# raymondclowe/EasyWakeWord

Hardware: AMD Instinct MI355X
Metric: real-time 16 kHz streams sustained + MFCC frames/sec at 1/2/4/8 GPUs (higher is better)
Workload: dtype fp32

## Files before the change

### easywakeword_amd/csrc/ewk_mfcc.hip

```cpp
#include <hip/hip_runtime.h>
#include <math.h>

#include "ewk_internal.h"
#include "ewk_score.h"
#include "ewk_db64.h"
#include "ewk_topdb_shift.h"
#include "ewk_rs_list.h"

#define EWK_SETPRIO(v) __builtin_amdgcn_s_setprio(v)

#ifdef EWK_TIMING
#define EWK_DBG_PARAM , uint64_t(&dbg)[kDbgN]
#define EWK_DBG_ARG , dbg
#define EWK_TS(v) const uint64_t v = __builtin_amdgcn_s_memtime()
#define EWK_TADD(k, a, b) dbg[k] += (b) - (a)
#define EWK_PASS_PARAM , uint64_t* pdbg
#define EWK_PASS_ARG(x) , x
#else
#define EWK_DBG_PARAM
#define EWK_DBG_ARG
#define EWK_TS(v)
#define EWK_TADD(k, a, b)
#define EWK_PASS_PARAM
#define EWK_PASS_ARG(x)
#endif
#ifdef EWK_TIMING
constexpr int kDbgN = 24;
#endif

namespace ewk {

#ifdef EWK_TIMING
__device__ unsigned long long g_ewk_dbg[kDbgN];
#endif
#ifdef EWK_LIST_STATS
__device__ unsigned long long g_ewk_list[10];
#endif
#ifdef EWK_COOP_DEBUG
constexpr int kCoopKeys = 32 * 256;
__device__ int4 g_coop_ev[kCoopKeys][WAVES];
__device__ float4 g_coop_th[kCoopKeys][WAVES];
__device__ double g_coop_pd[kCoopKeys][WAVES][60];
__device__ float g_coop_ms[kCoopKeys][40];
__device__ uint4 g_coop_tile[4 * 256][WAVES][512];
#define EWK_COOP_KEY_PARAM , int dkey
#define EWK_COOP_KEY_ARG(k) , (k)
#else
#define EWK_COOP_KEY_PARAM
#define EWK_COOP_KEY_ARG(k)
#endif

typedef float floatx4 __attribute__((ext_vector_type(4)));

constexpr int kFPP = 4 * kNF;
constexpr int kStageLoads = ((kFPP - 1) * HOP + NFFT + 63) / 64;
constexpr int kScrFrames = kFPP * SCR_FRAME + 8 * (kNF - 1);
__host__ __device__ constexpr int stg_off(int c) { return 256 * c + 128 * (c / 5); }
__host__ __device__ constexpr int win_off(int g, int n1) {
    return 4 * (160 * g + 32 * n1 + 32 * ((160 * g + 32 * n1) / 320));
}
constexpr int kStageFloats = stg_off(kStageLoads) / 4;
constexpr int kScrFloats = (kScrFrames > kStageFloats) ? kScrFrames : kStageFloats;
constexpr int SCR_BYTES = (kScrFloats * 4 + 15) & ~15;
constexpr int L_SCR = 0;
constexpr int L_TAB = L_SCR + WAVES * SCR_BYTES;
static_assert(L_SCR + (WAVES - 1) * SCR_BYTES < 65536, "ds_write_addtid_b32 bases must fit M0[15:0]");

constexpr int TP = 18;
constexpr int WP = 52;
constexpr int L_WIN2 = L_TAB;
constexpr int L_TW1 = L_WIN2 + 16 * TP * 8;
constexpr int L_TW2 = L_TW1 + 16 * TP * 8;
constexpr int L_WPAD = L_TW2 + 16 * TP * 8;
constexpr int L_BLO = L_WPAD + 16 * WP * 4;
constexpr int L_DCT = L_BLO + NMEL * 4;
constexpr float kDctScale = 1024.0f;
constexpr float kTopDbUnits = 80.0f;
constexpr int DCT_RT1 = 4 * 2 * 64 * 16;
constexpr int DCT_RT1_STRIDE = 17 * 16;
constexpr int kSlots = 5;
constexpr int DCT_BYTES = DCT_RT1 + 8 * DCT_RT1_STRIDE;
constexpr int L_SHARED_END = ((L_DCT + DCT_BYTES) + 15) & ~15;
constexpr int W_TILE = 0;
constexpr int kSpecTiles = 48;
constexpr int W_SPEC = W_TILE + 16 * NMEL * 4;
constexpr int kSpecRun = (16 / kFPP) * kSpecTiles;
constexpr int kSpecOrder = kSpecRun + kSpecTiles;
constexpr int W_BYTES = W_SPEC + (kSpecOrder + kSpecTiles) * 4;
static_assert(W_BYTES % 16 == 0 && kSpecTiles <= 64, "per-wave LDS carve; one bit per recorded tile");
constexpr int L_WG = L_SHARED_END + WAVES * W_BYTES;
constexpr int LDS_BYTES = L_WG + 16 + 8 * WAVES;
#ifndef EWK_TINY_MEAN
#define EWK_TINY_MEAN 32.0
#endif
constexpr double kTinyMean = EWK_TINY_MEAN;
#ifndef EWK_NAN_MARGIN_A
#define EWK_NAN_MARGIN_A 0.5
#endif
constexpr double kNanMarginA = EWK_NAN_MARGIN_A;
constexpr double kNanMarginB = 0.05;
static_assert(LDS_BYTES <= 160 * 1024, "the workgroup must fit a CU's LDS");
static_assert(16 % kFPP == 0, "passes must tile the 16-frame log-mel tile");


__device__ __forceinline__ void lds_order() { asm volatile("" ::: "memory"); }

#define EWK_LD128(r, a, c) asm volatile("ds_read_b128 %0, %1 offset:%2" : "=v"(r[c]) : "v"(a), "i"(16 * (c)) : "memory")
#define EWK_LD128_8(r, addr)                                                                        \
    do {                                                                                           \
        const uint32_t _a = (addr);                                                                \
        EWK_LD128(r, _a, 0); EWK_LD128(r, _a, 1); EWK_LD128(r, _a, 2); EWK_LD128(r, _a, 3);         \
        EWK_LD128(r, _a, 4); EWK_LD128(r, _a, 5); EWK_LD128(r, _a, 6); EWK_LD128(r, _a, 7);         \
    } while (0)
#define EWK_WAIT_8(r)                                                                              \
    asm volatile("s_waitcnt lgkmcnt(0)" : "+v"(r[0]), "+v"(r[1]), "+v"(r[2]), "+v"(r[3]), "+v"(r[4]), \
                 "+v"(r[5]), "+v"(r[6]), "+v"(r[7]) : : "memory")

__device__ __forceinline__ float2 cmul(float2 a, float2 w) {
    return make_float2(a.x * w.x - a.y * w.y, a.x * w.y + a.y * w.x);
}

__device__ __forceinline__ void dft4(float2& a0, float2& a1, float2& a2, float2& a3) {
    const float2 t0 = make_float2(a0.x + a2.x, a0.y + a2.y);
    const float2 t1 = make_float2(a0.x - a2.x, a0.y - a2.y);
    const float2 t2 = make_float2(a1.x + a3.x, a1.y + a3.y);
    const float2 t3 = make_float2(a1.x - a3.x, a1.y - a3.y);
    a0 = make_float2(t0.x + t2.x, t0.y + t2.y);
    a2 = make_float2(t0.x - t2.x, t0.y - t2.y);
    a1 = make_float2(t1.x + t3.y, t1.y - t3.x);
    a3 = make_float2(t1.x - t3.y, t1.y + t3.x);
}

__device__ __forceinline__ void dft16_stage2(float2 (&x)[16]) {
    constexpr float C1 = 0.92387953251128674f, R2 = 0.70710678118654752f, T = 0.41421356237309505f;
    dft4(x[0], x[1], x[2], x[3]);
    {
        const float2 a0 = x[4], y1 = x[5], y2 = x[6], y3 = x[7];
        const float2 u2 = make_float2(y2.x + y2.y, y2.y - y2.x);
        const float2 t0 = make_float2(fmaf(R2, u2.x, a0.x), fmaf(R2, u2.y, a0.y));
        const float2 t1 = make_float2(fmaf(-R2, u2.x, a0.x), fmaf(-R2, u2.y, a0.y));
        const float2 u1 = make_float2(fmaf(T, y1.y, y1.x), fmaf(-T, y1.x, y1.y));
        const float2 u3 = make_float2(fmaf(T, y3.x, y3.y), fmaf(T, y3.y, -y3.x));
        const float2 v2 = make_float2(u1.x + u3.x, u1.y + u3.y), v3 = make_float2(u1.x - u3.x, u1.y - u3.y);
        x[4] = make_float2(fmaf(C1, v2.x, t0.x), fmaf(C1, v2.y, t0.y));
        x[6] = make_float2(fmaf(-C1, v2.x, t0.x), fmaf(-C1, v2.y, t0.y));
        x[5] = make_float2(fmaf(C1, v3.y, t1.x), fmaf(-C1, v3.x, t1.y));
        x[7] = make_float2(fmaf(-C1, v3.y, t1.x), fmaf(C1, v3.x, t1.y));
    }
    {
        const float2 a0 = x[8], y1 = x[9], y2 = x[10], y3 = x[11];
        const float2 t0 = make_float2(a0.x + y2.y, a0.y - y2.x);
        const float2 t1 = make_float2(a0.x - y2.y, a0.y + y2.x);
        const float2 u1 = make_float2(y1.x + y1.y, y1.y - y1.x);
        const float d3 = y3.y - y3.x, n3 = y3.x + y3.y;
        const float2 v2 = make_float2(u1.x + d3, u1.y - n3), v3 = make_float2(u1.x - d3, u1.y + n3);
        x[8] = make_float2(fmaf(R2, v2.x, t0.x), fmaf(R2, v2.y, t0.y));
        x[10] = make_float2(fmaf(-R2, v2.x, t0.x), fmaf(-R2, v2.y, t0.y));
        x[9] = make_float2(fmaf(R2, v3.y, t1.x), fmaf(-R2, v3.x, t1.y));
        x[11] = make_float2(fmaf(-R2, v3.y, t1.x), fmaf(R2, v3.x, t1.y));
    }
    {
        const float2 a0 = x[12], y1 = x[13], y2 = x[14], y3 = x[15];
        const float d2 = y2.y - y2.x, n2 = y2.x + y2.y;
        const float2 t0 = make_float2(fmaf(R2, d2, a0.x), fmaf(-R2, n2, a0.y));
        const float2 t1 = make_float2(fmaf(-R2, d2, a0.x), fmaf(R2, n2, a0.y));
        const float2 u1 = make_float2(fmaf(T, y1.x, y1.y), fmaf(T, y1.y, -y1.x));
        const float m3 = fmaf(T, y3.y, y3.x), u3y = fmaf(T, y3.x, -y3.y);
        const float2 v2 = make_float2(u1.x - m3, u1.y + u3y), v3 = make_float2(u1.x + m3, u1.y - u3y);
        x[12] = make_float2(fmaf(C1, v2.x, t0.x), fmaf(C1, v2.y, t0.y));
        x[14] = make_float2(fmaf(-C1, v2.x, t0.x), fmaf(-C1, v2.y, t0.y));
        x[13] = make_float2(fmaf(C1, v3.y, t1.x), fmaf(-C1, v3.x, t1.y));
        x[15] = make_float2(fmaf(-C1, v3.y, t1.x), fmaf(C1, v3.x, t1.y));
    }
}

__device__ __forceinline__ void dft16_perm(float2 (&x)[16]) {
#pragma unroll
    for (int n2 = 0; n2 < 4; ++n2) dft4(x[n2], x[4 + n2], x[8 + n2], x[12 + n2]);
    dft16_stage2(x);
}
// ... 295 lines not shown
                    }
                }
            }
            lds_order();
        }
    }
    EWK_TS(fp3);
    EWK_SETPRIO(0);
#pragma unroll
    for (int g = 0; g < kNF; ++g) dft16_perm(b[g]);
    EWK_TS(fp4);
    {
        const bool z0 = jp == 0;
        float2 tw[18];
        {
            const float4* t4 = reinterpret_cast<const float4*>(smem + L_TW2) + jp * (TP / 2);
#pragma unroll
            for (int c = 0; c < 9; ++c) {
                const float4 q = t4[c];
                tw[2 * c] = make_float2(q.x, q.y);
                tw[2 * c + 1] = make_float2(q.z, q.w);
            }
        }
        float* pA0 = scf + rowA;
        float* pA1 = z0 ? scf - 136 : pA0;
        float* pA2 = z0 ? scf - 136 : pA0 - 16;
        float* pB0 = scf - rowA;
        float* pB1 = z0 ? scf + 136 : pB0;
        float* pB2 = z0 ? scf + 136 : pB0 + 16;
#pragma unroll
        for (int it0 = 0; it0 < 17; it0 += 2) {
            float py[2], px[2];
#pragma unroll
            for (int u = 0; u < 2; ++u) {
                const int it = it0 + u;
                if (it >= 17) break;
                const float2 w = tw[it];
                const float2 ug = b[0][dperm(it < 16 ? it : 15)];
                const float2 vg = b[1][dperm(it < 16 ? 15 - it : 0)];
                float2 uu, vv;
                if (it <= 8) {
                    uu = ug;
                    const float2 vz = b[0][dperm((16 - it) & 15)];
                    vv = z0 ? vz : vg;
                } else {
                    const float2 uz = b[1][dperm(it - 9)], vz = b[1][dperm(24 - it)];
                    uu = z0 ? uz : ug;
                    vv = z0 ? vz : vg;
                }
                const float ar = uu.x + vv.x, ai = uu.y - vv.y;
                const float br = uu.x - vv.x, bi = uu.y + vv.y;
                const float er = fmaf(w.y, br, -bi), ei = fmaf(w.y, bi, br);
                const float yr = fmaf(-w.x, er, ar), yi = fmaf(-w.x, ei, ai);
                const float xr = fmaf(w.x, er, ar), xi = fmaf(w.x, ei, ai);
                py[u] = yr * yr + yi * yi;
                px[u] = xr * xr + xi * xi;
            }
#pragma unroll
            for (int u = 0; u < 2; ++u) {
                const int it = it0 + u;
                if (it >= 17) break;
                float* pa = it <= 8 ? pA0 : (it < 16 ? pA1 : pA2);
                pa[16 * it] = py[u];
            }
#pragma unroll
            for (int u = 0; u < 2; ++u) {
                const int it = it0 + u;
                if (it >= 17) break;
                float* pb = it <= 8 ? pB0 : (it < 16 ? pB1 : pB2);
                pb[256 - 16 * it] = px[u];
            }
        }
        scf[257 + jp] = 0.0f;
        if (jp < 7) scf[265 + jp] = 0.0f;
    }
    lds_order();
    EWK_TS(fp5);
    EWK_SETPRIO(1);
    if (next_t0 >= 0) stage_load(v, next_t0 * HOP - NFFT / 2, lane, pf);
    float db[kNF][8];
    {
        const float* wrow = reinterpret_cast<const float*>(smem + L_WPAD) + j * WP;
#pragma unroll
        for (int hh = 0; hh < 2; ++hh) {
            const int i0 = hh ? 6 : 0, i1 = hh ? 8 : 6;
            float wv[MEL_ITERS], pv[kNF][MEL_ITERS];
#pragma unroll
            for (int i = i0; i < i1; ++i) {
                if (kMelW[i] <= 2) {
                    const float2 w = *reinterpret_cast<const float2*>(wrow + kMelOff[i]);
                    wv[kMelIt0[i]] = w.x; wv[kMelIt0[i] + 1] = w.y;
                } else {
#pragma unroll
                    for (int c = 0; c < (kMelW[i] + 3) / 4; ++c) {
                        const float4 w = *reinterpret_cast<const float4*>(wrow + kMelOff[i] + 4 * c);
                        const float ww[4] = {w.x, w.y, w.z, w.w};
#pragma unroll
                        for (int e = 0; e < 4; ++e)
                            if (4 * c + e < kMelW[i]) wv[kMelIt0[i] + 4 * c + e] = ww[e];
                    }
                }
#pragma unroll
                for (int g = 0; g < kNF; ++g) {
                    const float* sp = sc[g] + lo[i];
#pragma unroll
                    for (int q = 0; q < kMelW[i]; ++q) pv[g][kMelIt0[i] + q] = sp[q];
                }
            }
#pragma unroll
            for (int i = i0; i < i1; ++i)
#pragma unroll
                for (int g = 0; g < kNF; ++g) {
                    float acc = 0.0f;
#pragma unroll
                    for (int q = 0; q < kMelW[i]; ++q) acc = fmaf(wv[kMelIt0[i] + q], pv[g][kMelIt0[i] + q], acc);
                    db[g][i] = 3.0102999566398120f * __log2f(fmaxf(1e-10f, acc));
                    if (i == 0) nanp = fmaf(acc, 0.0f, nanp);
                }
        }
    }
    EWK_SETPRIO(0);
    lds_order();
    EWK_TS(fp6);
#pragma unroll
    for (int g = 0; g < kNF; ++g) {
        const int r = row0 + 2 * f + g;
        float fmx = db[g][0], fmn = db[g][0], x[8];
#pragma unroll
        for (int i = 0; i < 8; ++i) {
            fmx = fmaxf(fmx, db[g][i]);
            fmn = fminf(fmn, db[g][i]);
            x[i] = fmaxf(db[g][i], clampv);
        }
        vmax = fmaxf(vmax, valid[g] ? fmx : -INFINITY);
        vmin = fminf(vmin, valid[g] ? fmn : INFINITY);
        uint4 hi, lo;
        split8(x, hi, lo);
        unsigned char* tb = reinterpret_cast<unsigned char*>(tile) + tile_chunk(r, j);
        *reinterpret_cast<uint4*>(tb) = hi;
        *reinterpret_cast<uint4*>(tb + 256) = lo;
    }
    lds_order();
    if (next_t0 >= 0) stage_store(scr, lane, pf);
    lds_order();
#ifdef EWK_TIMING
    EWK_TS(fp7);
    if (pdbg) {
        pdbg[12] += fp1 - fp0; pdbg[13] += fp2 - fp1; pdbg[14] += fp3 - fp2; pdbg[15] += fp4 - fp3;
        pdbg[16] += fp5 - fp4; pdbg[17] += fp6 - fp5; pdbg[18] += fp7 - fp6; pdbg[19] += 1;
    }
#endif
}

#define EWK_DCT_RD(dst, addr, off) asm volatile("ds_read_b128 %0, %1 offset:%2" : "=v"(dst) : "v"(addr), "i"(off) : "memory")
#define EWK_DCT_LOAD(p, q)                                                   \
    do {                                                                     \
        EWK_DCT_RD(Bh[p], bq[q], 0);                                         \
        EWK_DCT_RD(Bl[p], bq[q], 256);                                       \
        EWK_DCT_RD(A0h[p], a0, 2048 * (q));                                  \
        EWK_DCT_RD(A0l[p], a0, 2048 * (q) + 1024);                           \
        EWK_DCT_RD(A1h[p], a1, DCT_RT1_STRIDE * (2 * (q)));                  \
        EWK_DCT_RD(A1l[p], a1, DCT_RT1_STRIDE * (2 * (q) + 1));              \
    } while (0)
#define EWK_DCT_WAIT(p, n)                                                                               \
    asm volatile("s_waitcnt lgkmcnt(" #n ")"                                                             \
                 : "+v"(Bh[p]), "+v"(Bl[p]), "+v"(A0h[p]), "+v"(A0l[p]), "+v"(A1h[p]), "+v"(A1l[p]) \
                 :                                                                                       \
                 : "memory")
#define EWK_MF(a, b, acc) \
    acc = __builtin_amdgcn_mfma_f32_16x16x32_f16(__builtin_bit_cast(halfx8, a), __builtin_bit_cast(halfx8, b), acc, 0, 0, 0)
#define EWK_DCT_MFMA(p)                                                                        \
    do {                                                                                       \
        EWK_MF(A0h[p], Bh[p], acc0); EWK_MF(A1h[p], Bh[p], acc1);                              \
        EWK_MF(A0h[p], Bl[p], acc0); EWK_MF(A1h[p], Bl[p], acc1);                              \
        EWK_MF(A0l[p], Bh[p], acc0); EWK_MF(A1l[p], Bh[p], acc1);                              \
        if (MASK) {                                                                            \
            const floatx4 mk = clamp_mask(Bh[p], Bl[p], cp, mnab);                             \
            EWK_MF(A0h[p], mk, am0); EWK_MF(A1h[p], mk, am1);                                  \
            EWK_MF(A0l[p], mk, am0); EWK_MF(A1l[p], mk, am1);                                  \
        }                                                                                      \
    } while (0)

__device__ __forceinline__ float pair_sum_lo(uint32_t h, uint32_t l) {
    float r;
    asm("v_fma_mix_f32 %0, %1, 1.0, %2 op_sel_hi:[1,0,1]" : "=v"(r) : "v"(h), "v"(l));
    return r;
}
__device__ __forceinline__ float pair_sum_hi(uint32_t h, uint32_t l) {
    float r;
    asm("v_fma_mix_f32 %0, %1, 1.0, %2 op_sel:[1,0,1] op_sel_hi:[1,0,1]" : "=v"(r) : "v"(h), "v"(l));
    return r;
}
struct ClampPair {
    uint32_t h2, l2;
    float eff;
};
__device__ __forceinline__ ClampPair clamp_pair(float clampv) {
    ClampPair cp;
    split2(clampv, clampv, cp.h2, cp.l2);
    cp.eff = pair_sum_lo(cp.h2, cp.l2);
    return cp;
}
__device__ __forceinline__ floatx4 clamp_mask(floatx4 bh, floatx4 bl, const ClampPair& cp, float& mn) {
    const uint4 h = __builtin_bit_cast(uint4, bh), l = __builtin_bit_cast(uint4, bl);
    const uint32_t hw[4] = {h.x, h.y, h.z, h.w}, lw[4] = {l.x, l.y, l.z, l.w};
    const uint32_t ones = 0x00010001u;
    uint32_t mw[4];
#pragma unroll
    for (int k = 0; k < 4; ++k) {
        const uint32_t t = (hw[k] ^ cp.h2) | (lw[k] ^ cp.l2);
        uint32_t u, zm;
        asm("v_pk_min_u16 %0, %1, %2" : "=v"(u) : "v"(t), "s"(ones));
        asm("v_pk_sub_u16 %0, %1, %2" : "=v"(zm) : "v"(u), "s"(ones));
        mw[k] = zm & 0x3C003C00u;
        const uint32_t hm = (zm & 0x7C007C00u) | (hw[k] & ~zm);
        asm("v_min3_f32 %0, %0, %1, %2" : "+v"(mn) : "v"(pair_sum_lo(hm, lw[k])), "v"(pair_sum_hi(hm, lw[k])));
    }
    return __builtin_bit_cast(floatx4, make_uint4(mw[0], mw[1], mw[2], mw[3]));
}

template <bool MASK>
__device__ __forceinline__ void tile_dct_m(const float* tile, const float* s_dct, int lane, float (&c)[kSlots],
                                           float (&m)[kSlots], float& mnab, const ClampPair& cp) {
    const int col = lane & 15, g4 = lane >> 4;
    floatx4 acc0 = {0.f, 0.f, 0.f, 0.f}, acc1 = {0.f, 0.f, 0.f, 0.f};
    floatx4 am0 = {0.f, 0.f, 0.f, 0.f}, am1 = {0.f, 0.f, 0.f, 0.f};
    const uint32_t tb = (uint32_t)(uintptr_t)tile + 512 * col + 16 * (g4 ^ (col & 3));
    uint32_t bq[4];
#pragma unroll
    for (int q = 0; q < 4; ++q) bq[q] = tb + 64 * (q ^ (col >> 2));
    const uint32_t db = (uint32_t)(uintptr_t)s_dct;
    const uint32_t a0 = db + 16 * lane;
    const uint32_t a1 = db + DCT_RT1 + 16 * ((col & 3) == 0 ? 4 * g4 + (col >> 2) : 16);
    floatx4 Bh[2], Bl[2], A0h[2], A0l[2], A1h[2], A1l[2];
    EWK_DCT_LOAD(0, 0);
    EWK_DCT_LOAD(1, 1);
    EWK_DCT_WAIT(0, 6);
    EWK_DCT_MFMA(0);
    EWK_DCT_LOAD(0, 2);
    EWK_DCT_WAIT(1, 6);
    EWK_DCT_MFMA(1);
    EWK_DCT_LOAD(1, 3);
    EWK_DCT_WAIT(0, 6);
    EWK_DCT_MFMA(0);
    EWK_DCT_WAIT(1, 0);
    EWK_DCT_MFMA(1);
    lds_order();
#pragma unroll
    for (int i = 0; i < 4; ++i) c[i] = acc0[i] * (1.0f / kDctScale);
    c[4] = acc1[0] * (1.0f / kDctScale);
    if (MASK) {
#pragma unroll
        for (int i = 0; i < 4; ++i) m[i] = am0[i] * (1.0f / kDctScale);
        m[4] = am1[0] * (1.0f / kDctScale);
    }
}
__device__ __forceinline__ void tile_dct(const float* tile, const float* s_dct, int lane, float (&c)[kSlots]) {
    float m[kSlots], mnab = 0.0f;
    tile_dct_m<false>(tile, s_dct, lane, c, m, mnab, ClampPair{0u, 0u, 0.0f});
}
#undef EWK_DCT_RD
#undef EWK_DCT_LOAD
#undef EWK_DCT_WAIT
#undef EWK_DCT_MFMA
#undef EWK_MF

__device__ __forceinline__ void stats_add(const float (&c)[kSlots], const float (&cref)[kSlots], bool ok, double (&s1)[kSlots],
                                          double (&s2)[kSlots]) {
    if (ok) {
#pragma unroll
        for (int i = 0; i < kSlots; ++i) {
            const double d = (double)c[i] - (double)cref[i];
            s1[i] += d;
            s2[i] = fma(d, d, s2[i]);
        }
    }
}

__device__ __forceinline__ void stats_replace(const float (&cn)[kSlots], const float (&co)[kSlots], const float (&cref)[kSlots],
                                              bool ok, double (&s1)[kSlots], double (&s2)[kSlots]) {
    if (ok) {
#pragma unroll
        for (int i = 0; i < kSlots; ++i) {
            const double dn = (double)cn[i] - (double)cref[i], dd = (double)co[i] - (double)cref[i];
            s1[i] += dn - dd;
            s2[i] += fma(dn, dn, -dd * dd);
        }
    }
}

__device__ __forceinline__ void shift_tile_add(const float (&c)[kSlots], const float (&cref)[kSlots],
                                               const float (&m)[kSlots], bool ok, float (&sA)[kSlots],
                                               float (&sB)[kSlots], float (&sC)[kSlots]) {
    if (ok) {
#pragma unroll
        for (int i = 0; i < kSlots; ++i) shift_add<float, float>(c[i] - cref[i], m[i], sA[i], sB[i], sC[i]);
    }
}
__device__ __forceinline__ void shift_apply(double delta, const float (&sA)[kSlots], float (&sB)[kSlots],
                                            const float (&sC)[kSlots], double (&s1)[kSlots], double (&s2)[kSlots]) {
#pragma unroll
    for (int i = 0; i < kSlots; ++i) shift_rise<float, float>(delta, sA[i], sB[i], sC[i], s1[i], s2[i]);
}
__device__ __forceinline__ void stats_replace_shift(const float (&cn)[kSlots], const float (&co)[kSlots], const float (&m)[kSlots],
                                                    double delta, const float (&cref)[kSlots], bool ok, double (&s1)[kSlots],
                                                    double (&s2)[kSlots]) {
    if (ok) {
#pragma unroll
        for (int i = 0; i < kSlots; ++i)
            shift_replace((double)cn[i], (double)co[i], (double)m[i], delta, (double)cref[i], s1[i], s2[i]);
    }
}

__device__ __forceinline__ void pass_mins(float x, float (&pm)[2]) {
    x = fminf(x, __int_as_float(__builtin_amdgcn_update_dpp(__float_as_int(x), __float_as_int(x), 0x111, 0xf, 0xf, false)));
    x = fminf(x, __int_as_float(__builtin_amdgcn_update_dpp(__float_as_int(x), __float_as_int(x), 0x112, 0xf, 0xf, false)));
    x = fminf(x, __int_as_float(__builtin_amdgcn_update_dpp(__float_as_int(x), __float_as_int(x), 0x114, 0xf, 0xf, false)));
#pragma unroll
    for (int p = 0; p < 2; ++p) {
        const float r0 = __int_as_float(__builtin_amdgcn_readlane(__float_as_int(x), 7 + 8 * p));
        const float r1 = __int_as_float(__builtin_amdgcn_readlane(__float_as_int(x), 23 + 8 * p));
        const float r2 = __int_as_float(__builtin_amdgcn_readlane(__float_as_int(x), 39 + 8 * p));
        const float r3 = __int_as_float(__builtin_amdgcn_readlane(__float_as_int(x), 55 + 8 * p));
        pm[p] = fminf(fminf(r0, r1), fminf(r2, r3));
    }
}

__device__ __forceinline__ float wave_min(float x) {
    x = fminf(x, __int_as_float(__builtin_amdgcn_update_dpp(__float_as_int(x), __float_as_int(x), 0x111, 0xf, 0xf, false)));
    x = fminf(x, __int_as_float(__builtin_amdgcn_update_dpp(__float_as_int(x), __float_as_int(x), 0x112, 0xf, 0xf, false)));
    x = fminf(x, __int_as_float(__builtin_amdgcn_update_dpp(__float_as_int(x), __float_as_int(x), 0x114, 0xf, 0xf, false)));
    x = fminf(x, __int_as_float(__builtin_amdgcn_update_dpp(__float_as_int(x), __float_as_int(x), 0x118, 0xf, 0xf, false)));
    const float r0 = __int_as_float(__builtin_amdgcn_readlane(__float_as_int(x), 15));
    const float r1 = __int_as_float(__builtin_amdgcn_readlane(__float_as_int(x), 31));
    const float r2 = __int_as_float(__builtin_amdgcn_readlane(__float_as_int(x), 47));
    const float r3 = __int_as_float(__builtin_amdgcn_readlane(__float_as_int(x), 63));
    return fminf(fminf(r0, r1), fminf(r2, r3));
}

template <int CTRL>
__device__ __forceinline__ double dpp_d(double x) {
    const int lo = __builtin_amdgcn_update_dpp(0, __double2loint(x), CTRL, 0xf, 0xf, false);
    const int hi = __builtin_amdgcn_update_dpp(0, __double2hiint(x), CTRL, 0xf, 0xf, false);
    return __hiloint2double(hi, lo);
}

__device__ __forceinline__ double row_sum_d(double x) {
    x += dpp_d<0x111>(x);
    x += dpp_d<0x112>(x);
    x += dpp_d<0x114>(x);
    x += dpp_d<0x118>(x);
    return x;
}

__device__ __forceinline__ double wave_sum_d(double x) {
    x = row_sum_d(x);
    double t = 0.0;
#pragma unroll
    for (int r = 0; r < 4; ++r)
        t += __hiloint2double(__builtin_amdgcn_readlane(__double2hiint(x), 16 * r + 15),
                              __builtin_amdgcn_readlane(__double2loint(x), 16 * r + 15));
    return t;
}

__device__ __forceinline__ float wave_sum_f(float x) {
    x += __int_as_float(__builtin_amdgcn_update_dpp(0, __float_as_int(x), 0x111, 0xf, 0xf, false));
    x += __int_as_float(__builtin_amdgcn_update_dpp(0, __float_as_int(x), 0x112, 0xf, 0xf, false));
    x += __int_as_float(__builtin_amdgcn_update_dpp(0, __float_as_int(x), 0x114, 0xf, 0xf, false));
    x += __int_as_float(__builtin_amdgcn_update_dpp(0, __float_as_int(x), 0x118, 0xf, 0xf, false));
    return (__int_as_float(__builtin_amdgcn_readlane(__float_as_int(x), 15)) +
            __int_as_float(__builtin_amdgcn_readlane(__float_as_int(x), 31))) +
           (__int_as_float(__builtin_amdgcn_readlane(__float_as_int(x), 47)) +
            __int_as_float(__builtin_amdgcn_readlane(__float_as_int(x), 63)));
}

__device__ __forceinline__ float wave_max(float x) { return -wave_min(-x); }

__device__ __forceinline__ void finish_stats(int T, const float (&cref)[kSlots], double (&s1)[kSlots], double (&s2)[kSlots],
                                             int lane, double* pd) {
#pragma unroll
    for (int i = 0; i < kSlots; ++i) {
        s1[i] = row_sum_d(s1[i]);
        s2[i] = row_sum_d(s2[i]);
    }
    if ((lane & 15) == 15) {
        const int h = lane >> 4;
#pragma unroll
        for (int r = 0; r < 4; ++r) {
            const int k = 4 * h + r;
            pd[3 * k] = s1[r]; pd[3 * k + 1] = s2[r]; pd[3 * k + 2] = (double)cref[r];
        }
        const int k2 = 16 + h;
        pd[3 * k2] = s1[4]; pd[3 * k2 + 1] = s2[4]; pd[3 * k2 + 2] = (double)cref[4];
    }
    lds_order();
    if (lane < NMFCC) {
        const double S1 = pd[3 * lane], S2 = pd[3 * lane + 1], r0 = pd[3 * lane + 2];
        const double Td = (double)T;
        const double mean = r0 + S1 / Td;
        double var = (S2 - S1 * S1 / Td) / Td;
        var = var > 0.0 ? var : 0.0;
        s1[0] = mean;
        s2[0] = sqrt(var);
    }
    lds_order();
}

__device__ __forceinline__ void zero_rows(float* tile, int row0, int lane) {
    for (int m = lane; m < kFPP * NMEL; m += 64) tile[row0 * NMEL + m] = 0.0f;
}

constexpr int kPassesPerTile = 16 / kFPP;
constexpr int kAllPasses = (1 << kPassesPerTile) - 1;
template <int RING>
__device__ __forceinline__ void tile_passes(const SegSrc<RING>& v, int tile_i, int T, const unsigned char* smem,
                                            float* scr, float* tile, int lane, const int (&lo)[8], float& mx,
                                            float& mn, float& nanp, float clampv, int mask = kAllPasses) {
    const int npass = (T + kFPP - 1) / kFPP;
    const int p0 = tile_i * kPassesPerTile;
    mask &= npass - p0 >= kPassesPerTile ? kAllPasses : (1 << max(0, npass - p0)) - 1;
    if (mask) {
        float r[kStageLoads];
        stage_load(v, (p0 + __builtin_ctz(mask)) * kFPP * HOP - NFFT / 2, lane, r);
        stage_store(scr, lane, r);
        lds_order();
    }
#pragma unroll 1
    for (int p = 0; p < kPassesPerTile; ++p) {
        if ((mask >> p) & 1) {
            const int rest = mask >> (p + 1);
            frame_pass(v, (p0 + p) * kFPP, T, p * kFPP, rest ? (p0 + p + 1 + __builtin_ctz(rest)) * kFPP : -1,
                       smem, scr, tile, lane, lo, mx, mn, nanp, clampv EWK_PASS_ARG(nullptr));
        } else {
            zero_rows(tile, p * kFPP, lane);
        }
    }
    lds_order();
}

template <int RING>
__device__ __forceinline__ void fix_tile(const SegSrc<RING>& v, int tile_i, int T, float run, float theta,
                                         const unsigned char* smem, float* scr, float* tile, int lane,
                                         const int (&lo)[8], const float (&cref)[kSlots], double (&s1)[kSlots],
                                         double (&s2)[kSlots], int mask = kAllPasses, bool shifted = false) {
    const float* s_dct = reinterpret_cast<const float*>(smem + L_DCT);
    float d0 = 0.f, d1 = 0.f, d2 = 0.f;
    tile_passes(v, tile_i, T, smem, scr, tile, lane, lo, d0, d1, d2, run, mask);
    float co[kSlots], cn[kSlots], m[kSlots];
    const ClampPair cp = clamp_pair(run), ct = clamp_pair(theta);
    if (shifted) tile_dct_m<true>(tile, s_dct, lane, co, m, d0, cp);
    else tile_dct(tile, s_dct, lane, co);
    {
        uint4 h[4], l[4];
        clamp_load(reinterpret_cast<const float4*>(tile), lane, h, l);
        clamp_store(tile, lane, h, l, theta);
    }
    lds_order();
    tile_dct(tile, s_dct, lane, cn);
    const int col = lane & 15;
    const bool ok = tile_i * 16 + col < T && ((mask >> (col / kFPP)) & 1);
    if (shifted) stats_replace_shift(cn, co, m, (double)ct.eff - (double)cp.eff, cref, ok, s1, s2);
    else stats_replace(cn, co, cref, ok, s1, s2);
}

constexpr int kScoutBatch = 8;
template <int RING, int NB>
__device__ __forceinline__ void scout_batch(const SegSrc<RING>& v, int t0, int lane, float& e) {
    float x[NB][4];
#pragma unroll
    for (int u = 0; u < NB; ++u) {
#pragma unroll
        for (int q = 0; q < 4; ++q) {
            const int qs = (t0 + u) * 16 * HOP + 640 * q + 64 + lane;
            int off;
            if (RING) {
                const int phys = qs >= v.wrap_at ? qs - v.wrap_at : qs + v.start;
                off = (unsigned)qs < (unsigned)v.len ? phys * sample_bytes(RING) : -1;
            } else {
                off = qs * 4;
            }
            if (RING == 2)
                x[u][q] = (float)(short)__builtin_amdgcn_raw_buffer_load_b16(v.rsrc, off, 0, 0);
            else
                x[u][q] = __builtin_bit_cast(float, __builtin_amdgcn_raw_buffer_load_b32(v.rsrc, off, 0, 0));
        }
    }
#pragma unroll
    for (int u = 0; u < NB; ++u) {
        float a = x[u][0] * x[u][0];
#pragma unroll
        for (int q = 1; q < 4; ++q) a = fmaf(x[u][q], x[u][q], a);
        const float tot = wave_sum_f(a);
        if (lane == t0 + u) e = tot;
    }
}

template <int RING>
__device__ __forceinline__ float scout_tiles(const SegSrc<RING>& v, int ntile, int lane) {
    float e = -1.0f;
    for (int t0 = 0; t0 < ntile; t0 += kScoutBatch) {
        const int left = ntile - t0;
        if (left <= 2) scout_batch<RING, 2>(v, t0, lane, e);
        else if (left <= 4) scout_batch<RING, 4>(v, t0, lane, e);
        else scout_batch<RING, kScoutBatch>(v, t0, lane, e);
    }
    return e;
}

struct WorkAhead {
    int state = 0;
    bool first = true;
    int idx = 0;
    int seg = 0;
    int64_t start = 0;
    int32_t len = 0;
    int32_t stream = 0;
    int32_t flags = 0;
};
struct WorkCtx {
    const ScoreArgs* a;
    int base, count;
    bool ahead;
    int wid, nw;
};

template <int RING>
__device__ __forceinline__ void work_claim(const WorkCtx& c, WorkAhead& w, int lane) {
    if (w.first) {
        w.idx = c.wid;
        w.first = false;
    } else if (lane == 0) {
        w.idx = c.nw + atomicAdd(c.a->work, 1);
    }
    w.state = 1;
}
template <int RING>
__device__ __forceinline__ void work_order(const WorkCtx& c, WorkAhead& w) {
    w.idx = __shfl(w.idx, 0, 64);
    w.state = 2;
    if (w.idx < c.count) w.seg = c.base + ((!RING && c.a->order) ? c.a->order[w.idx] : w.idx);
}
template <int RING>
__device__ __forceinline__ void work_describe(const WorkCtx& c, WorkAhead& w) {
    w.state = 3;
    if (w.idx >= c.count) return;
    if (RING) {
        const ewk_event ev = c.a->events[w.seg];
        w.start = ev.ring_start;
        w.len = ev.length;
        w.stream = ev.stream;
        w.flags = ev.flags;
    } else {
        w.start = c.a->offsets[w.seg];
        w.len = c.a->lengths[w.seg];
    }
}

template <int RING>
__device__ void segment_stats(const SegSrc<RING>& v, const unsigned char* smem, float* scr, float* tile,
                              float* spec, int lane, const int (&lo)[8], double (&s1)[kSlots], double (&s2)[kSlots],
                              float& theta_out, const WorkCtx& wc, WorkAhead& nx EWK_DBG_PARAM) {
    EWK_TS(tq0);
    const float* s_dct = reinterpret_cast<const float*>(smem + L_DCT);
    const int T = 1 + v.len / HOP;
    const int ntile = (T + 15) >> 4;
    const int npass = (T + kFPP - 1) / kFPP;
    const int col = lane & 15;
    int* order = reinterpret_cast<int*>(spec + kSpecOrder);
    const bool ordered = ntile > 1 && ntile <= kSpecTiles;
    if (ordered) {
        float e = scout_tiles(v, ntile, lane);
        e = e == e ? e : 0.0f;
        int rank = 0;
        for (int u = 0; u < ntile; ++u) {
            const float eu = __int_as_float(__builtin_amdgcn_readlane(__float_as_int(e), u));
            rank += (eu > e) || (eu == e && u < lane);
        }
        if (lane < ntile) order[rank] = lane;
        lds_order();
    }
    EWK_TS(tq1);
    EWK_TADD(1, tq0, tq1);
    float cref[kSlots];
#pragma unroll
    for (int i = 0; i < kSlots; ++i) { s1[i] = 0.0; s2[i] = 0.0; cref[i] = 0.0f; }
    float vmax = -INFINITY, nanp = 0.0f;
    int tile_i = ordered ? order[0] : 0;
    {
        float r[kStageLoads];
        stage_load(v, tile_i * 16 * HOP - NFFT / 2, lane, r);
        stage_store(scr, lane, r);
        lds_order();
    }
    EWK_TS(tq2);
    EWK_TADD(2, tq1, tq2);
    float run = -INFINITY;
    static_assert(kPassesPerTile == 2, "pass_mins splits a tile in two passes");
    float srun = -INFINITY, amin = INFINITY;
    int nshift = 0;
    float sA[kSlots], sB[kSlots], sC[kSlots];
#pragma unroll
    for (int i = 0; i < kSlots; ++i) { sA[i] = 0.0f; sB[i] = 0.0f; sC[i] = 0.0f; }
    uint64_t shifted = 0;
    for (int k = 0; k < ntile; ++k) {
        EWK_TS(tk0);
        const int next_tile = k + 1 < ntile ? (ordered ? order[k + 1] : k + 1) : -1;
        const bool rec = tile_i < kSpecTiles;
        float tmw = INFINITY;
        if (!rec) run = -INFINITY;
        const bool last = k + 1 == ntile;
        if (last && wc.ahead) work_claim<RING>(wc, nx, lane);
#pragma unroll 1
        for (int p = 0; p < kPassesPerTile; ++p) {
            const int pass = tile_i * kPassesPerTile + p;
            const int nxt = p + 1 < kPassesPerTile && pass + 1 < npass ? (pass + 1) * kFPP
                                                                      : (next_tile >= 0 ? next_tile * 16 : -1);
            float tp = INFINITY;
            if (pass < npass)
                frame_pass(v, pass * kFPP, T, p * kFPP, nxt, smem, scr, tile, lane, lo, vmax, tp, nanp, run EWK_PASS_ARG(dbg));
            else
                zero_rows(tile, p * kFPP, lane);
            const float tpw = wave_min(tp);
            tmw = fminf(tmw, tpw);
            if (lane == 0 && rec) spec[kPassesPerTile * tile_i + p] = tpw;
        }
        lds_order();
        EWK_TS(tk1);
        EWK_TADD(3, tk0, tk1);
        if (last && wc.ahead) work_order<RING>(wc, nx);
        const float run2 = rec ? wave_max(vmax) - kTopDbUnits : -INFINITY;
        if (run2 > run && tmw < run2) {
            uint4 h[4], l[4];
            clamp_load(reinterpret_cast<const float4*>(tile), lane, h, l);
            clamp_store(tile, lane, h, l, run2);
            lds_order();
        }
        run = fmaxf(run, run2);
        if (rec) {
            if (nshift && run > srun) shift_apply((double)clamp_pair(run).eff - (double)clamp_pair(srun).eff, sA, sB, sC, s1, s2);
            srun = run;
        }
        const bool masked = rec && tmw < run;
        const bool ok = tile_i * 16 + col < T;
        float c[kSlots], m[kSlots], mnab = INFINITY;
        EWK_TS(tm0);
        if (masked) tile_dct_m<true>(tile, s_dct, lane, c, m, mnab, clamp_pair(run));
        else tile_dct(tile, s_dct, lane, c);
        EWK_TS(tm1);
        if (k == 0) {
#pragma unroll
            for (int i = 0; i < kSlots; ++i) cref[i] = __shfl(c[i], lane & 48, 64);
        }
        stats_add(c, cref, ok, s1, s2);
        float pm[kPassesPerTile] = {INFINITY, INFINITY};
        EWK_TS(tm3);
        if (masked) {
            shift_tile_add(c, cref, m, ok, sA, sB, sC);
            nshift = 1;
            shifted |= 1ull << tile_i;
            pass_mins(ok ? mnab : INFINITY, pm);
            amin = fminf(amin, fminf(pm[0], pm[1]));
#ifdef EWK_TIMING
            EWK_TS(tm2);
            dbg[20] += 1;
            dbg[21] += (tm1 - tm0) + (tm2 - tm3);
#endif
        } else {
            amin = fminf(amin, fmaxf(tmw, run));
        }
        if (lane == 0 && rec) {
#pragma unroll
            for (int p = 0; p < kPassesPerTile; ++p)
                spec[kPassesPerTile * tile_i + p] = masked ? pm[p] : fmaxf(spec[kPassesPerTile * tile_i + p], run);
            spec[kSpecRun + tile_i] = run;
        }
        tile_i = next_tile;
        EWK_TS(tk2);
        EWK_TADD(4, tk1, tk2);
#ifdef EWK_TIMING
        if (!masked) { dbg[22] += tm1 - tm0; dbg[23] += 1; }
#endif
    }
    EWK_TS(tq3);
    if (wc.ahead) work_describe<RING>(wc, nx);
    vmax = wave_max(vmax);
    const float theta = vmax - kTopDbUnits;
    theta_out = theta;
    if (nshift && theta > srun) shift_apply((double)clamp_pair(theta).eff - (double)clamp_pair(srun).eff, sA, sB, sC, s1, s2);
    if (amin < theta) {
        lds_order();
        for (int cur = 0; cur < ntile; ++cur) {
            const bool rec = cur < kSpecTiles;
            int mask = kAllPasses;
            if (rec) {
                mask = 0;
#pragma unroll
                for (int p = 0; p < kPassesPerTile; ++p) mask |= (shift_flags<float>(spec[kPassesPerTile * cur + p], theta) ? 1 : 0) << p;
                if (!mask) continue;
            }
#ifdef EWK_TIMING
            dbg[10] += 1;
            dbg[11] += __builtin_popcount(mask);
#endif
            fix_tile(v, cur, T, rec ? spec[kSpecRun + cur] : -INFINITY, theta, smem, scr, tile, lane, lo, cref, s1,
                     s2, mask, rec && ((shifted >> cur) & 1));
        }
    }
    if (__ballot(nanp != nanp)) {
#pragma unroll
        for (int i = 0; i < kSlots; ++i) s1[i] = __builtin_nan("");
    }
    EWK_TS(tq4);
    EWK_TADD(5, tq3, tq4);
#ifndef EWK_SKIP_EPI
    finish_stats(T, cref, s1, s2, lane, reinterpret_cast<double*>(scr));
#endif
    EWK_TS(tq5);
    EWK_TADD(6, tq4, tq5);
}


template <int RING>
__device__ void segment_stats_coop(const SegSrc<RING>& v, unsigned char* smem, float* scr, float* tile,
                                   float* spec, int wave, int lane, const int (&lo)[8], float* misc0,
                                   float& theta_out EWK_COOP_KEY_PARAM) {
    const float* s_dct = reinterpret_cast<const float*>(smem + L_DCT);
    float* wg_mm = reinterpret_cast<float*>(smem + L_WG + 16);
    const int T = 1 + v.len / HOP;
    const int ntile = (T + 15) >> 4;
    const int nloc = ntile > wave ? (ntile - wave + WAVES - 1) / WAVES : 0;
    const int col = lane & 15;
    double s1[kSlots], s2[kSlots];
    float cref[kSlots];
#pragma unroll
    for (int i = 0; i < kSlots; ++i) { s1[i] = 0.0; s2[i] = 0.0; cref[i] = 0.0f; }
    float vmax = -INFINITY, vmin = INFINITY, nanp = 0.0f;
    float run = -INFINITY, last_min = INFINITY;
    for (int lt = 0; lt < nloc; ++lt) {
        const int tile_i = wave + WAVES * lt;
        const bool last = lt + 1 == nloc;
        const bool rec = !last && lt < kSpecTiles;
        if (!rec) run = -INFINITY;
        float tmin = INFINITY;
        tile_passes(v, tile_i, T, smem, scr, tile, lane, lo, vmax, tmin, nanp, run);
        const float tmw = wave_min(tmin);
        vmin = fminf(vmin, tmw);
#ifdef EWK_COOP_DEBUG
        if (last && dkey < 4 * 256) {
            lds_order();
#pragma unroll
            for (int u = 0; u < 8; ++u) g_coop_tile[dkey][wave][64 * u + lane] = reinterpret_cast<const uint4*>(tile)[64 * u + lane];
        }
#endif
        if (last) { last_min = tmw; break; }
        const float run2 = rec ? wave_max(vmax) - kTopDbUnits : -INFINITY;
        if (run2 > run && tmw < run2) {
            uint4 h[4], l[4];
            clamp_load(reinterpret_cast<const float4*>(tile), lane, h, l);
            clamp_store(tile, lane, h, l, run2);
            lds_order();
        }
        run = fmaxf(run, run2);
        float c[kSlots];
        tile_dct(tile, s_dct, lane, c);
        if (lt == 0) {
#pragma unroll
            for (int i = 0; i < kSlots; ++i) cref[i] = __shfl(c[i], lane & 48, 64);
        }
        stats_add(c, cref, tile_i * 16 + col < T, s1, s2);
        if (lane == 0 && rec) {
#pragma unroll
            for (int p = 0; p < kPassesPerTile; ++p) spec[kPassesPerTile * lt + p] = fmaxf(tmw, run);
            spec[kSpecRun + lt] = run;
        }
    }
    vmax = wave_max(vmax);
    if (lane == 0) { wg_mm[2 * wave] = vmax; wg_mm[2 * wave + 1] = vmin; }
    __syncthreads();
#pragma unroll
    for (int w = 0; w < WAVES; ++w) { vmax = fmaxf(vmax, wg_mm[2 * w]); vmin = fminf(vmin, wg_mm[2 * w + 1]); }
    const float theta = vmax - kTopDbUnits;
    theta_out = theta;
#ifdef EWK_COOP_DEBUG
    if (lane == 0) g_coop_th[dkey][wave] = make_float4(wg_mm[2 * wave], wg_mm[2 * wave + 1], theta, (float)nloc);
#endif
    if (nloc > 0) {
        const int tile_l = wave + WAVES * (nloc - 1);
        if (last_min < theta) {
            uint4 h[4], l[4];
            clamp_load(reinterpret_cast<const float4*>(tile), lane, h, l);
            clamp_store(tile, lane, h, l, theta);
            lds_order();
        }
        float c[kSlots];
        tile_dct(tile, s_dct, lane, c);
        if (nloc == 1) {
#pragma unroll
            for (int i = 0; i < kSlots; ++i) cref[i] = __shfl(c[i], lane & 48, 64);
        }
        stats_add(c, cref, tile_l * 16 + col < T, s1, s2);
        if (vmin < theta) {
            lds_order();
            for (int lt = 0; lt + 1 < nloc; ++lt) {
                const bool rec = lt < kSpecTiles;
                if (rec && !(spec[kPassesPerTile * lt] < theta)) continue;
                fix_tile(v, wave + WAVES * lt, T, rec ? spec[kSpecRun + lt] : -INFINITY, theta, smem, scr, tile,
                         lane, lo, cref, s1, s2);
            }
        }
    }
    if (__ballot(nanp != nanp)) {
#pragma unroll
        for (int i = 0; i < kSlots; ++i) s1[i] = __builtin_nan("");
    }
    double* pd = reinterpret_cast<double*>(scr);
#pragma unroll
    for (int i = 0; i < kSlots; ++i) { s1[i] = row_sum_d(s1[i]); s2[i] = row_sum_d(s2[i]); }
    if (col == 15) {
        const int h = lane >> 4;
#pragma unroll
        for (int r = 0; r < 4; ++r) {
            const int k = 4 * h + r;
            pd[3 * k] = s1[r]; pd[3 * k + 1] = s2[r]; pd[3 * k + 2] = (double)cref[r];
        }
        const int k2 = 16 + h;
        pd[3 * k2] = s1[4]; pd[3 * k2 + 1] = s2[4]; pd[3 * k2 + 2] = (double)cref[4];
    }
    __syncthreads();
#ifdef EWK_COOP_DEBUG
    if (lane < 60) g_coop_pd[dkey][wave][lane] = pd[lane];
#endif
    if (wave == 0) {
        double mean = 0.0, sd = 0.0;
// ... 462 lines not shown
```

Measured before the change: 2.863 billion.

## Prefetch DCT operands before reductions and interleave mask computation with MFMAs

```diff
diff --git a/easywakeword_amd/csrc/ewk_mfcc.hip b/easywakeword_amd/csrc/ewk_mfcc.hip
--- a/easywakeword_amd/csrc/ewk_mfcc.hip
+++ b/easywakeword_amd/csrc/ewk_mfcc.hip
@@ -16,6 +16,8 @@
 #define EWK_TADD(k, a, b) dbg[k] += (b) - (a)
 #define EWK_PASS_PARAM , uint64_t* pdbg
 #define EWK_PASS_ARG(x) , x
+#define EWK_ISSUE_PARAM , uint64_t* t_issue = nullptr
+#define EWK_ISSUE_ARG(x) , x
 #else
 #define EWK_DBG_PARAM
 #define EWK_DBG_ARG
@@ -23,9 +25,11 @@
 #define EWK_TADD(k, a, b)
 #define EWK_PASS_PARAM
 #define EWK_PASS_ARG(x)
+#define EWK_ISSUE_PARAM
+#define EWK_ISSUE_ARG(x)
 #endif
 #ifdef EWK_TIMING
-constexpr int kDbgN = 24;
+constexpr int kDbgN = 28;
 #endif
 
 namespace ewk {
@@ -627,32 +631,58 @@
 #endif
 }
 
+struct DctOps {
+    floatx4 Bh[4], Bl[4], A0h[4], A0l[4], A1h[4], A1l[4];
+};
+#define EWK_DCT_OPS(o)                                                                             \
+    floatx4(&Bh)[4] = o.Bh, (&Bl)[4] = o.Bl, (&A0h)[4] = o.A0h, (&A0l)[4] = o.A0l, (&A1h)[4] = o.A1h, \
+    (&A1l)[4] = o.A1l
 #define EWK_DCT_RD(dst, addr, off) asm volatile("ds_read_b128 %0, %1 offset:%2" : "=v"(dst) : "v"(addr), "i"(off) : "memory")
-#define EWK_DCT_LOAD(p, q)                                                   \
+#define EWK_DCT_LOAD(q)                                                      \
     do {                                                                     \
-        EWK_DCT_RD(Bh[p], bq[q], 0);                                         \
-        EWK_DCT_RD(Bl[p], bq[q], 256);                                       \
-        EWK_DCT_RD(A0h[p], a0, 2048 * (q));                                  \
-        EWK_DCT_RD(A0l[p], a0, 2048 * (q) + 1024);                           \
-        EWK_DCT_RD(A1h[p], a1, DCT_RT1_STRIDE * (2 * (q)));                  \
-        EWK_DCT_RD(A1l[p], a1, DCT_RT1_STRIDE * (2 * (q) + 1));              \
+        EWK_DCT_RD(Bh[q], bq[q], 0);                                         \
+        EWK_DCT_RD(Bl[q], bq[q], 256);                                       \
+        EWK_DCT_RD(A0h[q], a0, 2048 * (q));                                  \
+        EWK_DCT_RD(A0l[q], a0, 2048 * (q) + 1024);                           \
+        EWK_DCT_RD(A1h[q], a1, DCT_RT1_STRIDE * (2 * (q)));                  \
+        EWK_DCT_RD(A1l[q], a1, DCT_RT1_STRIDE * (2 * (q) + 1));              \
     } while (0)
-#define EWK_DCT_WAIT(p, n)                                                                               \
-    asm volatile("s_waitcnt lgkmcnt(" #n ")"                                                             \
-                 : "+v"(Bh[p]), "+v"(Bl[p]), "+v"(A0h[p]), "+v"(A0l[p]), "+v"(A1h[p]), "+v"(A1l[p]) \
-                 :                                                                                       \
-                 : "memory")
+#define EWK_DCT_WAIT(q, n)                                                                                   \
+    do {                                                                                                     \
+        __builtin_amdgcn_sched_barrier(0);                                                                   \
+        asm volatile("s_waitcnt lgkmcnt(" #n ")"                                                             \
+                     : "+v"(Bh[q]), "+v"(Bl[q]), "+v"(A0h[q]), "+v"(A0l[q]), "+v"(A1h[q]), "+v"(A1l[q]) \
+                     :                                                                                       \
+                     : "memory");                                                                            \
+        __builtin_amdgcn_sched_barrier(0);                                                                   \
+    } while (0)
 #define EWK_MF(a, b, acc) \
     acc = __builtin_amdgcn_mfma_f32_16x16x32_f16(__builtin_bit_cast(halfx8, a), __builtin_bit_cast(halfx8, b), acc, 0, 0, 0)
-#define EWK_DCT_MFMA(p)                                                                        \
+#define EWK_MKW(q, k) \
+    mw[q][k] = clamp_mask_word(__float_as_uint(Bh[q][k]), __float_as_uint(Bl[q][k]), cp, mnab)
+#define EWK_MK(q) __builtin_bit_cast(floatx4, make_uint4(mw[q][0], mw[q][1], mw[q][2], mw[q][3]))
+#define EWK_DCT_STEP(q)                                                                        \
     do {                                                                                       \
-        EWK_MF(A0h[p], Bh[p], acc0); EWK_MF(A1h[p], Bh[p], acc1);                              \
-        EWK_MF(A0h[p], Bl[p], acc0); EWK_MF(A1h[p], Bl[p], acc1);                              \
-        EWK_MF(A0l[p], Bh[p], acc0); EWK_MF(A1l[p], Bh[p], acc1);                              \
+        constexpr int qm = (q) > 0 ? (q) - 1 : 0;                                              \
+        EWK_MF(A0h[q], Bh[q], acc0); EWK_MF(A1h[q], Bh[q], acc1);                              \
+        if (MASK) EWK_MKW(q, 0);                                                               \
+        EWK_MF(A0h[q], Bl[q], acc0); EWK_MF(A1h[q], Bl[q], acc1);                              \
+        if (MASK) EWK_MKW(q, 1);                                                               \
+        EWK_MF(A0l[q], Bh[q], acc0); EWK_MF(A1l[q], Bh[q], acc1);                              \
+        if (MASK) EWK_MKW(q, 2);                                                               \
+        if (MASK && (q) > 0) { EWK_MF(A0h[qm], EWK_MK(qm), am0); EWK_MF(A1h[qm], EWK_MK(qm), am1); } \
+        if (MASK) EWK_MKW(q, 3);                                                               \
+        if (MASK && (q) > 0) { EWK_MF(A0l[qm], EWK_MK(qm), am0); EWK_MF(A1l[qm], EWK_MK(qm), am1); } \
+         \
+                    \
+        asm volatile("" : "+v"(acc0), "+v"(acc1));                                             \
+        if (MASK && (q) > 0) asm volatile("" : "+v"(am0), "+v"(am1));                          \
+    } while (0)
+#define EWK_DCT_TAIL(q)                                                                        \
+    do {                                                                                       \
         if (MASK) {                                                                            \
-            const floatx4 mk = clamp_mask(Bh[p], Bl[p], cp, mnab);                             \
-            EWK_MF(A0h[p], mk, am0); EWK_MF(A1h[p], mk, am1);                                  \
-            EWK_MF(A0l[p], mk, am0); EWK_MF(A1l[p], mk, am1);                                  \
+            EWK_MF(A0h[q], EWK_MK(q), am0); EWK_MF(A1h[q], EWK_MK(q), am1);                    \
+            EWK_MF(A0l[q], EWK_MK(q), am0); EWK_MF(A1l[q], EWK_MK(q), am1);                    \
         }                                                                                      \
     } while (0)
 
@@ -676,50 +706,74 @@
     cp.eff = pair_sum_lo(cp.h2, cp.l2);
     return cp;
 }
-__device__ __forceinline__ floatx4 clamp_mask(floatx4 bh, floatx4 bl, const ClampPair& cp, float& mn) {
-    const uint4 h = __builtin_bit_cast(uint4, bh), l = __builtin_bit_cast(uint4, bl);
-    const uint32_t hw[4] = {h.x, h.y, h.z, h.w}, lw[4] = {l.x, l.y, l.z, l.w};
+__device__ __forceinline__ uint32_t clamp_mask_word(uint32_t hw, uint32_t lw, const ClampPair& cp, float& mn) {
     const uint32_t ones = 0x00010001u;
-    uint32_t mw[4];
-#pragma unroll
-    for (int k = 0; k < 4; ++k) {
-        const uint32_t t = (hw[k] ^ cp.h2) | (lw[k] ^ cp.l2);
-        uint32_t u, zm;
-        asm("v_pk_min_u16 %0, %1, %2" : "=v"(u) : "v"(t), "s"(ones));
-        asm("v_pk_sub_u16 %0, %1, %2" : "=v"(zm) : "v"(u), "s"(ones));
-        mw[k] = zm & 0x3C003C00u;
-        const uint32_t hm = (zm & 0x7C007C00u) | (hw[k] & ~zm);
-        asm("v_min3_f32 %0, %0, %1, %2" : "+v"(mn) : "v"(pair_sum_lo(hm, lw[k])), "v"(pair_sum_hi(hm, lw[k])));
-    }
-    return __builtin_bit_cast(floatx4, make_uint4(mw[0], mw[1], mw[2], mw[3]));
-}
-
-template <bool MASK>
-__device__ __forceinline__ void tile_dct_m(const float* tile, const float* s_dct, int lane, float (&c)[kSlots],
-                                           float (&m)[kSlots], float& mnab, const ClampPair& cp) {
+    const uint32_t t = (hw ^ cp.h2) | (lw ^ cp.l2);
+    uint32_t u, zm;
+    asm("v_pk_min_u16 %0, %1, %2" : "=v"(u) : "v"(t), "s"(ones));
+    asm("v_pk_sub_u16 %0, %1, %2" : "=v"(zm) : "v"(u), "s"(ones));
+    const uint32_t hm = (zm & 0x7C007C00u) | (hw & ~zm);
+    asm("v_min3_f32 %0, %0, %1, %2" : "+v"(mn) : "v"(pair_sum_lo(hm, lw)), "v"(pair_sum_hi(hm, lw)));
+    return zm & 0x3C003C00u;
+}
+
+__device__ __forceinline__ void tile_dct_b_addr(const float* tile, int lane, uint32_t (&bq)[4]) {
     const int col = lane & 15, g4 = lane >> 4;
-    floatx4 acc0 = {0.f, 0.f, 0.f, 0.f}, acc1 = {0.f, 0.f, 0.f, 0.f};
-    floatx4 am0 = {0.f, 0.f, 0.f, 0.f}, am1 = {0.f, 0.f, 0.f, 0.f};
     const uint32_t tb = (uint32_t)(uintptr_t)tile + 512 * col + 16 * (g4 ^ (col & 3));
+#pragma unroll
+    for (int q = 0; q < 4; ++q) bq[q] = tb + 64 * (q ^ (col >> 2));
+}
+__device__ __forceinline__ void tile_dct_request(const float* tile, const float* s_dct, int lane, DctOps& o) {
+    const int col = lane & 15, g4 = lane >> 4;
     uint32_t bq[4];
-#pragma unroll
-    for (int q = 0; q < 4; ++q) bq[q] = tb + 64 * (q ^ (col >> 2));
+    tile_dct_b_addr(tile, lane, bq);
     const uint32_t db = (uint32_t)(uintptr_t)s_dct;
     const uint32_t a0 = db + 16 * lane;
     const uint32_t a1 = db + DCT_RT1 + 16 * ((col & 3) == 0 ? 4 * g4 + (col >> 2) : 16);
-    floatx4 Bh[2], Bl[2], A0h[2], A0l[2], A1h[2], A1l[2];
-    EWK_DCT_LOAD(0, 0);
-    EWK_DCT_LOAD(1, 1);
-    EWK_DCT_WAIT(0, 6);
-    EWK_DCT_MFMA(0);
-    EWK_DCT_LOAD(0, 2);
-    EWK_DCT_WAIT(1, 6);
-    EWK_DCT_MFMA(1);
-    EWK_DCT_LOAD(1, 3);
-    EWK_DCT_WAIT(0, 6);
-    EWK_DCT_MFMA(0);
+    EWK_DCT_OPS(o);
+    EWK_DCT_LOAD(0);
+    EWK_DCT_LOAD(1);
+    EWK_DCT_LOAD(2);
+    EWK_DCT_LOAD(3);
+}
+__device__ __forceinline__ void tile_dct_settle(DctOps& o) {
+    EWK_DCT_OPS(o);
+    EWK_DCT_WAIT(0, 0);
     EWK_DCT_WAIT(1, 0);
-    EWK_DCT_MFMA(1);
+    EWK_DCT_WAIT(2, 0);
+    EWK_DCT_WAIT(3, 0);
+}
+__device__ __forceinline__ void tile_dct_request_b(const float* tile, int lane, DctOps& o) {
+    uint32_t bq[4];
+    tile_dct_b_addr(tile, lane, bq);
+    EWK_DCT_OPS(o);
+#pragma unroll
+    for (int q = 0; q < 4; ++q) {
+        EWK_DCT_RD(Bh[q], bq[q], 0);
+        EWK_DCT_RD(Bl[q], bq[q], 256);
+    }
+    tile_dct_settle(o);
+}
+
+template <bool MASK>
+__device__ __forceinline__ void tile_dct_run(DctOps& o, float (&c)[kSlots], float (&m)[kSlots], float& mnab,
+                                             const ClampPair& cp EWK_ISSUE_PARAM) {
+    floatx4 acc0 = {0.f, 0.f, 0.f, 0.f}, acc1 = {0.f, 0.f, 0.f, 0.f};
+    floatx4 am0 = {0.f, 0.f, 0.f, 0.f}, am1 = {0.f, 0.f, 0.f, 0.f};
+    EWK_DCT_OPS(o);
+    uint32_t mw[4][4];
+    EWK_DCT_WAIT(0, 14);
+#ifdef EWK_TIMING
+    if (t_issue) *t_issue = __builtin_amdgcn_s_memtime();
+#endif
+    EWK_DCT_STEP(0);
+    EWK_DCT_WAIT(1, 12);
+    EWK_DCT_STEP(1);
+    EWK_DCT_WAIT(2, 6);
+    EWK_DCT_STEP(2);
+    EWK_DCT_WAIT(3, 0);
+    EWK_DCT_STEP(3);
+    EWK_DCT_TAIL(3);
     lds_order();
 #pragma unroll
     for (int i = 0; i < 4; ++i) c[i] = acc0[i] * (1.0f / kDctScale);
@@ -730,14 +784,25 @@
         m[4] = am1[0] * (1.0f / kDctScale);
     }
 }
-__device__ __forceinline__ void tile_dct(const float* tile, const float* s_dct, int lane, float (&c)[kSlots]) {
+template <bool MASK>
+__device__ __forceinline__ void tile_dct_m(const float* tile, const float* s_dct, int lane, float (&c)[kSlots],
+                                           float (&m)[kSlots], float& mnab, const ClampPair& cp EWK_ISSUE_PARAM) {
+    DctOps o;
+    tile_dct_request(tile, s_dct, lane, o);
+    tile_dct_run<MASK>(o, c, m, mnab, cp EWK_ISSUE_ARG(t_issue));
+}
+__device__ __forceinline__ void tile_dct(const float* tile, const float* s_dct, int lane, float (&c)[kSlots] EWK_ISSUE_PARAM) {
     float m[kSlots], mnab = 0.0f;
-    tile_dct_m<false>(tile, s_dct, lane, c, m, mnab, ClampPair{0u, 0u, 0.0f});
+    tile_dct_m<false>(tile, s_dct, lane, c, m, mnab, ClampPair{0u, 0u, 0.0f} EWK_ISSUE_ARG(t_issue));
 }
 #undef EWK_DCT_RD
 #undef EWK_DCT_LOAD
+#undef EWK_DCT_OPS
 #undef EWK_DCT_WAIT
-#undef EWK_DCT_MFMA
+#undef EWK_DCT_STEP
+#undef EWK_DCT_TAIL
+#undef EWK_MKW
+#undef EWK_MK
 #undef EWK_MF
 
 __device__ __forceinline__ void stats_add(const float (&c)[kSlots], const float (&cref)[kSlots], bool ok, double (&s1)[kSlots],
@@ -851,6 +916,26 @@
 
 __device__ __forceinline__ float wave_max(float x) { return -wave_min(-x); }
 
+__device__ __forceinline__ void wave_min3(float& a, float& b, float& c) {
+#define EWK_MIN_DPP(x, ctrl) \
+    x = fminf(x, __int_as_float(__builtin_amdgcn_update_dpp(__float_as_int(x), __float_as_int(x), ctrl, 0xf, 0xf, false)))
+    EWK_MIN_DPP(a, 0x111); EWK_MIN_DPP(b, 0x111); EWK_MIN_DPP(c, 0x111);
+    EWK_MIN_DPP(a, 0x112); EWK_MIN_DPP(b, 0x112); EWK_MIN_DPP(c, 0x112);
+    EWK_MIN_DPP(a, 0x114); EWK_MIN_DPP(b, 0x114); EWK_MIN_DPP(c, 0x114);
+    EWK_MIN_DPP(a, 0x118); EWK_MIN_DPP(b, 0x118); EWK_MIN_DPP(c, 0x118);
+#undef EWK_MIN_DPP
+    float r[3][4];
+#pragma unroll
+    for (int i = 0; i < 4; ++i) {
+        r[0][i] = __int_as_float(__builtin_amdgcn_readlane(__float_as_int(a), 16 * i + 15));
+        r[1][i] = __int_as_float(__builtin_amdgcn_readlane(__float_as_int(b), 16 * i + 15));
+        r[2][i] = __int_as_float(__builtin_amdgcn_readlane(__float_as_int(c), 16 * i + 15));
+    }
+    a = fminf(fminf(r[0][0], r[0][1]), fminf(r[0][2], r[0][3]));
+    b = fminf(fminf(r[1][0], r[1][1]), fminf(r[1][2], r[1][3]));
+    c = fminf(fminf(r[2][0], r[2][1]), fminf(r[2][2], r[2][3]));
+}
+
 __device__ __forceinline__ void finish_stats(int T, const float (&cref)[kSlots], double (&s1)[kSlots], double (&s2)[kSlots],
                                              int lane, double* pd) {
 #pragma unroll
@@ -859,7 +944,8 @@
         s2[i] = row_sum_d(s2[i]);
     }
     if ((lane & 15) == 15) {
-        const int h = lane >> 4;
+        int h = lane >> 4;
+        asm volatile("" : "+v"(h));
 #pragma unroll
         for (int r = 0; r < 4; ++r) {
             const int k = 4 * h + r;
@@ -1081,10 +1167,10 @@
         EWK_TS(tk0);
         const int next_tile = k + 1 < ntile ? (ordered ? order[k + 1] : k + 1) : -1;
         const bool rec = tile_i < kSpecTiles;
-        float tmw = INFINITY;
         if (!rec) run = -INFINITY;
         const bool last = k + 1 == ntile;
         if (last && wc.ahead) work_claim<RING>(wc, nx, lane);
+        float tpl[kPassesPerTile] = {INFINITY, INFINITY};
 #pragma unroll 1
         for (int p = 0; p < kPassesPerTile; ++p) {
             const int pass = tile_i * kPassesPerTile + p;
@@ -1095,20 +1181,26 @@
                 frame_pass(v, pass * kFPP, T, p * kFPP, nxt, smem, scr, tile, lane, lo, vmax, tp, nanp, run EWK_PASS_ARG(dbg));
             else
                 zero_rows(tile, p * kFPP, lane);
-            const float tpw = wave_min(tp);
-            tmw = fminf(tmw, tpw);
-            if (lane == 0 && rec) spec[kPassesPerTile * tile_i + p] = tpw;
+            if (p == 0) tpl[0] = tp;
+            else tpl[1] = tp;
         }
         lds_order();
         EWK_TS(tk1);
         EWK_TADD(3, tk0, tk1);
         if (last && wc.ahead) work_order<RING>(wc, nx);
-        const float run2 = rec ? wave_max(vmax) - kTopDbUnits : -INFINITY;
+        DctOps ops;
+        tile_dct_request(tile, s_dct, lane, ops);
+        float nvm = -vmax;
+        wave_min3(tpl[0], tpl[1], nvm);
+        const float tmw = fminf(tpl[0], tpl[1]);
+        const float run2 = rec ? -nvm - kTopDbUnits : -INFINITY;
         if (run2 > run && tmw < run2) {
+            tile_dct_settle(ops);
             uint4 h[4], l[4];
             clamp_load(reinterpret_cast<const float4*>(tile), lane, h, l);
             clamp_store(tile, lane, h, l, run2);
             lds_order();
+            tile_dct_request_b(tile, lane, ops);
         }
         run = fmaxf(run, run2);
         if (rec) {
@@ -1119,8 +1211,11 @@
         const bool ok = tile_i * 16 + col < T;
         float c[kSlots], m[kSlots], mnab = INFINITY;
         EWK_TS(tm0);
-        if (masked) tile_dct_m<true>(tile, s_dct, lane, c, m, mnab, clamp_pair(run));
-        else tile_dct(tile, s_dct, lane, c);
+#ifdef EWK_TIMING
+        uint64_t tmi = 0;
+#endif
+        if (masked) tile_dct_run<true>(ops, c, m, mnab, clamp_pair(run) EWK_ISSUE_ARG(&tmi));
+        else tile_dct_run<false>(ops, c, m, mnab, ClampPair{0u, 0u, 0.0f} EWK_ISSUE_ARG(&tmi));
         EWK_TS(tm1);
         if (k == 0) {
 #pragma unroll
@@ -1146,7 +1241,7 @@
         if (lane == 0 && rec) {
 #pragma unroll
             for (int p = 0; p < kPassesPerTile; ++p)
-                spec[kPassesPerTile * tile_i + p] = masked ? pm[p] : fmaxf(spec[kPassesPerTile * tile_i + p], run);
+                spec[kPassesPerTile * tile_i + p] = masked ? pm[p] : fmaxf(tpl[p], run);
             spec[kSpecRun + tile_i] = run;
         }
         tile_i = next_tile;
@@ -1154,6 +1249,7 @@
         EWK_TADD(4, tk1, tk2);
 #ifdef EWK_TIMING
         if (!masked) { dbg[22] += tm1 - tm0; dbg[23] += 1; }
+        dbg[24] += tm0 - tk1; dbg[25] += tmi - tm0; dbg[26] += tm1 - tmi; dbg[27] += tk2 - tm1;
 #endif
     }
     EWK_TS(tq3);
```

Result: no change. 2.870 billion, median of 5 (+0.2%).
